# MDAnalysis/transport-analysis

Measured on AMD Instinct MI355X. Metric: VACF lag-points/sec (n_frames x n_atoms / s), higher is better.
Workload: dtype f64

## Files before the change

transport_analysis_amd/csrc/wfft.hpp:

```cpp
#pragma once
#include <hip/hip_runtime.h>

#include <type_traits>
#include <utility>

#include "fft_engine.hpp"

namespace ta {

#ifndef WF_NW_R0
#define WF_NW_R0 0
#define WF_NW_VAL 0
#endif

template <int LO, int HI, class F>
__device__ __forceinline__ void static_for_range(F&& f) {
    [&]<int... I>(std::integer_sequence<int, I...>) {
        (f(std::integral_constant<int, LO + I>{}), ...);
    }(std::make_integer_sequence<int, (HI > LO ? HI - LO : 0)>{});
}

typedef unsigned int wf_u32x4 __attribute__((ext_vector_type(4)));

#include "wfft_twist.inc"
// ... 341 lines not shown
        for (int n2 = 0; n2 < 8; ++n2) v[n2] = reg[64 * n2 + lane];
    }
    __device__ __forceinline__ void stage_a(cd* __restrict__ reg, cd (&v)[8], const cd (&twa)[7]) const {
        Dft<8>::run(v);
#pragma unroll
        for (int a = 1; a < 8; ++a) v[a] = cmul(v[a], twa[a - 1]);
        __builtin_amdgcn_wave_barrier();
#pragma unroll
        for (int a = 0; a < 8; ++a) reg[a * 64 + (lane ^ (8 * (a & 1)))] = v[a];
        __builtin_amdgcn_wave_barrier();
        const int base = hi * 64 + (lo ^ (8 * (hi & 1)));
#pragma unroll
        for (int n1 = 0; n1 < 8; ++n1) v[n1] = reg[base ^ (8 * n1)];
        __builtin_amdgcn_wave_barrier();
    }
    __device__ __forceinline__ void stage_b(cd* __restrict__ reg, cd (&v)[8], const cd (&twb)[7]) const {
        Dft<8>::run(v);
#pragma unroll
        for (int b = 1; b < 8; ++b) v[b] = cmul(v[b], twb[b - 1]);
        __builtin_amdgcn_wave_barrier();
        const int x = lo ^ hi;
#pragma unroll
        for (int b = 0; b < 8; ++b) reg[(hi * 8 + b) * 8 + (x ^ b)] = v[b];
        __builtin_amdgcn_wave_barrier();
#pragma unroll
        for (int n0 = 0; n0 < 8; ++n0) v[n0] = reg[lane * 8 + (n0 ^ x)];
        __builtin_amdgcn_wave_barrier();
    }
    __device__ __forceinline__ void stage_c(cd (&v)[8], double (&acc)[8]) const {
        Dft<8>::run(v);
#pragma unroll
        for (int c = 0; c < 8; ++c) acc[c] = fma(v[c].y, v[c].y, fma(v[c].x, v[c].x, acc[c]));
        __builtin_amdgcn_wave_barrier();
    }
};

template <int ROT>
__device__ __forceinline__ void wf_bf(cd& A, cd& B, const cd t) {
    const double qx = fma(-t.x, B.y, B.x), qy = fma(t.x, B.x, B.y);
    const cd a = A;
    if constexpr (ROT == 0) {
        A = cd{fma(t.y, qx, a.x), fma(t.y, qy, a.y)};
        B = cd{fma(-t.y, qx, a.x), fma(-t.y, qy, a.y)};
    } else {
        A = cd{fma(t.y, qy, a.x), fma(-t.y, qx, a.y)};
        B = cd{fma(-t.y, qy, a.x), fma(t.y, qx, a.y)};
    }
}
__device__ __forceinline__ void wf_dft8_tw(cd (&v)[8], const cd (&t)[4]) {
    wf_bf<0>(v[0], v[4], t[0]);
    wf_bf<0>(v[1], v[5], t[0]);
    wf_bf<0>(v[2], v[6], t[0]);
    wf_bf<0>(v[3], v[7], t[0]);
    wf_bf<0>(v[0], v[2], t[1]);
    wf_bf<0>(v[1], v[3], t[1]);
    wf_bf<1>(v[4], v[6], t[1]);
    wf_bf<1>(v[5], v[7], t[1]);
    wf_bf<0>(v[0], v[1], t[2]);
    wf_bf<1>(v[2], v[3], t[2]);
    wf_bf<0>(v[4], v[5], t[3]);
    wf_bf<1>(v[6], v[7], t[3]);
    const cd y4 = v[1], y6 = v[3], y1 = v[4], y3 = v[6];
    v[1] = y1, v[3] = y3, v[4] = y4, v[6] = y6;
}

struct WfTw {
    cd b[4], c[4];
};
typedef unsigned wf_u32pair __attribute__((ext_vector_type(2)));
__device__ __forceinline__ void wf_transpose_hi(cd (&v)[8]) {
    unsigned w[8][4];
#pragma unroll
    for (int a = 0; a < 8; ++a) {
        const wf_u32x4 t = __builtin_bit_cast(wf_u32x4, v[a]);
        w[a][0] = t.x, w[a][1] = t.y, w[a][2] = t.z, w[a][3] = t.w;
    }
#pragma unroll
    for (int a = 0; a < 8; ++a)
        if (!(a & 4))
#pragma unroll
            for (int d = 0; d < 4; ++d) {
                const wf_u32pair r = __builtin_amdgcn_permlane32_swap(w[a][d], w[a | 4][d], false, false);
                w[a][d] = r.x, w[a | 4][d] = r.y;
            }
#pragma unroll
    for (int a = 0; a < 8; ++a)
        if (!(a & 2))
#pragma unroll
            for (int d = 0; d < 4; ++d) {
                const wf_u32pair r = __builtin_amdgcn_permlane16_swap(w[a][d], w[a | 2][d], false, false);
                w[a][d] = r.x, w[a | 2][d] = r.y;
            }
#pragma unroll
    for (int a = 0; a < 8; ++a)
        if (!(a & 1))
#pragma unroll
            for (int d = 0; d < 4; ++d) {
                const unsigned lo = w[a][d], hi = w[a | 1][d];
                w[a][d] = __builtin_amdgcn_update_dpp(lo, hi, 0x128, 0xF, 0xC, false);
                w[a | 1][d] = __builtin_amdgcn_update_dpp(hi, lo, 0x128, 0xF, 0x3, false);
            }
#pragma unroll
    for (int a = 0; a < 8; ++a) {
        wf_u32x4 t;
        t.x = w[a][0], t.y = w[a][1], t.z = w[a][2], t.w = w[a][3];
        v[a] = __builtin_bit_cast(cd, t);
    }
}

struct WfAddr {
    unsigned we, wo, re, ro, x16, b2w, b2r;
    __device__ __forceinline__ void init(int lane, unsigned q_bytes) {
        const int hi = lane >> 3, lo = lane & 7;
        we = q_bytes + 16u * (unsigned)lane;
        wo = q_bytes + 16u * (unsigned)(lane ^ 8);
        const unsigned rb = q_bytes + 16u * (unsigned)(hi * 64 + lo);
        re = rb + 128u * (unsigned)(hi & 1);
        ro = rb - 128u * (unsigned)(hi & 1);
        x16 = 16u * (unsigned)(hi ^ lo);
        b2w = q_bytes + 1024u * (unsigned)hi;
        b2r = b2w + 128u * (unsigned)lo;
    }
    __device__ __forceinline__ unsigned w2(int k) const { return (x16 ^ (16u * (unsigned)k)) + b2w; }
    __device__ __forceinline__ unsigned r2(int k) const { return (x16 ^ (16u * (unsigned)k)) + b2r; }
};
struct WfSub {
    const WfAddr& ad;
    unsigned char* smem;
    __device__ __forceinline__ WfSub(const WfAddr& ad_, unsigned char* smem_) : ad(ad_), smem(smem_) {}
    __device__ __forceinline__ cd& at(unsigned base, unsigned off) const {
        return *reinterpret_cast<cd*>(__builtin_assume_aligned(smem + (base + off), 16));
    }
    template <unsigned SO>
    __device__ __forceinline__ void read_a(cd (&v)[8]) const {
#pragma unroll
        for (int n2 = 0; n2 < 8; ++n2) v[n2] = at(ad.we, SO + 1024u * n2);
    }
    template <unsigned SO>
    __device__ __forceinline__ void stage_a_w(cd (&v)[8]) const {
        Dft<8>::run(v);
        __builtin_amdgcn_wave_barrier();
#pragma unroll
        for (int a = 0; a < 8; ++a) at(a & 1 ? ad.wo : ad.we, SO + 1024u * a) = v[a];
        __builtin_amdgcn_wave_barrier();
    }
    template <unsigned SO>
    __device__ __forceinline__ void stage_a_r(cd (&v)[8]) const {
        __builtin_amdgcn_wave_barrier();
#pragma unroll
        for (int n1 = 0; n1 < 8; ++n1) v[n1] = at(n1 & 1 ? ad.ro : ad.re, SO + 128u * n1);
        __builtin_amdgcn_wave_barrier();
    }
    template <unsigned SO, bool XV = false>
    __device__ __forceinline__ void stage_a(cd (&v)[8]) const {
        if constexpr (XV) {
            Dft<8>::run(v);
            wf_transpose_hi(v);
        } else {
            stage_a_w<SO>(v);
            stage_a_r<SO>(v);
        }
    }
    template <unsigned SO>
    __device__ __forceinline__ void stage_b_w(cd (&v)[8], const WfTw& tw) const {
        wf_dft8_tw(v, tw.b);
        __builtin_amdgcn_wave_barrier();
#pragma unroll
        for (int b = 0; b < 8; ++b) at(ad.w2(b), SO + 128u * b) = v[b];
        __builtin_amdgcn_wave_barrier();
    }
    template <unsigned SO>
    __device__ __forceinline__ void stage_b_r(cd (&v)[8]) const {
        __builtin_amdgcn_wave_barrier();
#pragma unroll
        for (int n0 = 0; n0 < 8; ++n0) v[n0] = at(ad.r2(n0), SO);
        __builtin_amdgcn_wave_barrier();
    }
    template <unsigned SO>
    __device__ __forceinline__ void stage_b(cd (&v)[8], const WfTw& tw) const {
        stage_b_w<SO>(v, tw);
        stage_b_r<SO>(v);
    }
    __device__ __forceinline__ void stage_c(cd (&v)[8], const WfTw& tw, double (&acc)[8]) const {
        wf_dft8_tw(v, tw.c);
#pragma unroll
        for (int c = 0; c < 8; ++c) acc[c] = fma(v[c].y, v[c].y, fma(v[c].x, v[c].x, acc[c]));
    }
    __device__ __forceinline__ void stage_c_w(cd (&v)[8], const WfTw& tw, double (&acc)[8], double wgt) const {
        wf_dft8_tw(v, tw.c);
#pragma unroll
        for (int c = 0; c < 8; ++c) acc[c] = fma(wgt, fma(v[c].y, v[c].y, v[c].x * v[c].x), acc[c]);
    }
};

constexpr unsigned kWfSubBytes = 512 * sizeof(cd);

struct WfNoHook {
    template <class T>
    __device__ __forceinline__ void operator()(T) const {}
};
template <int I>
using wf_part = std::integral_constant<int, I>;

template <int S0, bool XV = false, class Hook = WfNoHook>
__device__ __forceinline__ void wf_sub512(const WfSub& w, const WfTw& tw, double (&acc)[8], Hook&& hook = Hook{}) {
    cd v[8];
    w.read_a<S0 * kWfSubBytes>(v);
    hook(wf_part<0>{});
    w.template stage_a<S0 * kWfSubBytes, XV>(v);
    hook(wf_part<1>{});
    w.stage_b<S0 * kWfSubBytes>(v, tw);
    hook(wf_part<2>{});
    w.stage_c(v, tw, acc);
    hook(wf_part<3>{});
}

template <int S0, bool XV = false>
__device__ __forceinline__ void wf_sub512_w(const WfSub& w, const WfTw& tw, double (&acc)[8], double wgt) {
    cd v[8];
    w.read_a<S0 * kWfSubBytes>(v);
    w.template stage_a<S0 * kWfSubBytes, XV>(v);
    w.stage_b<S0 * kWfSubBytes>(v, tw);
    w.stage_c_w(v, tw, acc, wgt);
}

template <int S0, bool XV = false, class Hook = WfNoHook>
__device__ __forceinline__ void wf_sub512_x2(const WfSub& w, const WfTw& tw, double (&acc0)[8],
                                             double (&acc1)[8], Hook&& hook = Hook{}) {
    constexpr unsigned A = S0 * kWfSubBytes, B = A + kWfSubBytes;
    cd v0[8], v1[8];
    w.read_a<A>(v0);
    w.read_a<B>(v1);
    __builtin_amdgcn_wave_barrier();
    hook(wf_part<0>{});
    w.template stage_a<A>(v0);
    w.template stage_a<B, XV>(v1);
    hook(wf_part<1>{});
    w.stage_b<A>(v0, tw);
    w.stage_b<B>(v1, tw);
    hook(wf_part<2>{});
    w.stage_c(v0, tw, acc0);
    w.stage_c(v1, tw, acc1);
    hook(wf_part<3>{});
}

template <bool XV = false, class Hook = WfNoHook>
__device__ __forceinline__ void wf_sub512_x3(const WfSub& w, const WfTw& tw, double (&acc0)[8],
                                             double (&acc1)[8], double (&acc2)[8], Hook&& hook = Hook{}) {
    constexpr unsigned A = 0, B = kWfSubBytes, C = 2 * kWfSubBytes;
    cd v0[8], v1[8], v2[8];
    w.read_a<A>(v0);
    w.read_a<B>(v1);
    w.read_a<C>(v2);
    __builtin_amdgcn_wave_barrier();
    hook(wf_part<0>{});
    w.template stage_a<A>(v0);
    w.template stage_a<B>(v1);
    w.template stage_a<C, XV>(v2);
    hook(wf_part<1>{});
    w.stage_b<A>(v0, tw);
    w.stage_b<B>(v1, tw);
    w.stage_b<C>(v2, tw);
    hook(wf_part<2>{});
    w.stage_c(v0, tw, acc0);
    w.stage_c(v1, tw, acc1);
    w.stage_c(v2, tw, acc2);
    hook(wf_part<3>{});
}

__device__ __forceinline__ void wf_unit_of(long atom, int k, int D, long* pair, int* kind) {
    const long c0 = atom * D;
    if (D == 2) {
        *pair = atom, *kind = 2;
    } else if (D == 1) {
        *pair = c0 >> 1, *kind = (int)(c0 & 1);
    } else if ((c0 & 1) == 0) {
        *pair = (c0 >> 1) + k, *kind = k == 0 ? 2 : 0;
    } else {
        *pair = (c0 >> 1) + k, *kind = k == 0 ? 1 : 2;
    }
}

typedef unsigned int wf_u32x2 __attribute__((__vector_size__(2 * sizeof(unsigned int))));

__device__ __forceinline__ cd wf_cfma(cd acc, cd a, cd b) {
    return {acc.x + (a.x * b.x - a.y * b.y), acc.y + (a.x * b.y + a.y * b.x)};
}

template <bool S, class A, class B>
__device__ __forceinline__ auto& wf_pick(A& a, B& b) {
    if constexpr (S) return a;
    else return b;
}

#ifndef WF_PASS_SPLIT
#define WF_PASS_SPLIT 1
#endif
#ifndef WF_SEED_DERIVE
#define WF_SEED_DERIVE 2
#endif
#ifndef WF_TWIST_FOLD
#define WF_TWIST_FOLD 1
#endif
template <class P, bool BYP, bool LONG, bool SRC32>
constexpr bool wf_pass_split = WF_PASS_SPLIT && !BYP && !LONG && !SRC32 && (P::R0 == 18 || P::R0 == 20);

__device__ __forceinline__ cd wf_csqr(cd a) { return {a.x * a.x - a.y * a.y, 2.0 * (a.x * a.y)}; }

template <class P, bool BYP, bool LONG, bool STAMP, bool SRC32, int PASS>
__device__ __forceinline__ void wf_accum_body(unsigned char* smem_raw, const double* __restrict__ pm, long pitch, int T,
                                              long n_units, const cd* __restrict__ tw2, double* __restrict__ accg, int D,
                                              int R_arg, unsigned long long* __restrict__ stamps) {
    cd* lds = reinterpret_cast<cd*>(smem_raw);
    constexpr int R0 = P::R0, N1 = P::N1, NW = P::NW, NS1 = P::NS1, M = P::M;
    static_assert(!(SRC32 && LONG), "float32 slabs: plans without an outer radix only");
    static_assert(PASS < 0 || (!BYP && !LONG), "a compile-time pass: lag sums without an outer radix");
    const int R = LONG ? R_arg : 1, npass = 2 * R, L = npass * M;
    const int tid = threadIdx.x, wave = tid >> 6;
    int lane = tid & 63;
    const int bi = blockIdx.x >> 3;
    const int pass = PASS >= 0 ? PASS : bi % npass;
    constexpr bool kTwistFold = PASS == 1 && WF_TWIST_FOLD && DftTwisted<R0>::kHave;
    const long tuple = (blockIdx.x & 7) + 8 * (bi / npass), n_tuples = gridDim.x / npass;
    const int upa = BYP ? (D == 3 ? 2 : 1) : 1;
    const int grp = BYP && (D & 1) ? 2 : 1;

    double acc[NS1][8];
#pragma unroll
    for (int s = 0; s < NS1; ++s)
#pragma unroll
        for (int c = 0; c < 8; ++c) acc[s][c] = 0.0;
    unsigned long long st_acc[4] = {0, 0, 0, 0}, st_prev = 0, st_t0 = 0, st_r0 = 0, st_tail = 0, st_s2end = 0;
    if constexpr (STAMP) {
        st_prev = st_t0 = __builtin_amdgcn_s_memtime();
        st_r0 = __builtin_amdgcn_s_memrealtime();
    }
#define WF_STAMP(i)                                                   \
    if constexpr (STAMP) {                                            \
        const unsigned long long now_ = __builtin_amdgcn_s_memtime(); \
        st_acc[i] += now_ - st_prev;                                  \
        st_prev = now_;                                               \
    }
    const __amdgpu_buffer_rsrc_t twr =
        __builtin_amdgcn_make_buffer_rsrc(const_cast<cd*>(tw2), 0, (L + kWfStageRows * 64) * 16, 0x00020000);
    auto unit_rsrc = [&](long item, int k, int* kind) {
        long pair = item;
        const bool live = item < n_units;
        *kind = 2;
        if constexpr (BYP) wf_unit_of(live ? item : 0, k, D, &pair, kind);
        if constexpr (SRC32)
            return __builtin_amdgcn_make_buffer_rsrc(
                const_cast<float*>(reinterpret_cast<const float*>(pm) + (live ? pair : 0) * pitch * 2), 0,
                live ? T * 8 : 0, 0x00020000);
        else
            return __builtin_amdgcn_make_buffer_rsrc(const_cast<double*>(pm + (live ? pair : 0) * pitch * 2), 0,
                                                     live ? T * 16 : 0, 0x00020000);
    };
    using RowT = std::conditional_t<SRC32, wf_u32x2, cd>;
    auto load_row = [&](__amdgpu_buffer_rsrc_t rs, int kd, int u, unsigned row_off) -> RowT {
        if constexpr (SRC32) {
            return __builtin_amdgcn_raw_buffer_load_b64(rs, (unsigned)u * 8u, row_off * 8u, 0);
        } else {
            if (!BYP || kd == 2) return wf_load(rs, (unsigned)u * 16u, row_off * 16u);
            return cd{__builtin_bit_cast(double, __builtin_amdgcn_raw_buffer_load_b64(
                                                     rs, (unsigned)u * 16u + (unsigned)kd * 8u, row_off * 16u, 0)),
                      0.0};
        }
    };
    [[maybe_unused]] auto wf_widen = [&](wf_u32x2 r, int kd) {
        if (!BYP || kd == 2)
            return cd{(double)__builtin_bit_cast(float, (unsigned)r[0]), (double)__builtin_bit_cast(float, (unsigned)r[1])};
        return cd{(double)__builtin_bit_cast(float, (unsigned)(kd ? r[1] : r[0])), 0.0};
    };
    constexpr int K1 = P::K1, NT = P::NT;
    RowT xx[K1][R0];
    auto issue_loads = [&](__amdgpu_buffer_rsrc_t rs, int kd) {
#pragma unroll
        for (int k1 = 0; k1 < K1; ++k1) {
            const int u = tid + NT * k1;
            if (K1 * NT != N1 && u >= N1) continue;
            if (!BYP || kd == 2) {
#pragma unroll
                for (int j = 0; j < R0; ++j) xx[k1][j] = load_row(rs, 2, u, (unsigned)(N1 * j));
            } else {
#pragma unroll
                for (int j = 0; j < R0; ++j) xx[k1][j] = load_row(rs, kd, u, (unsigned)(N1 * j));
            }
        }
    };
#ifndef WF_LOAD_PARTS
#define WF_LOAD_PARTS 4
#endif
    constexpr int NR = K1 * R0;
    constexpr bool kSpread = P::kSpreadRows || (SRC32 && R0 >= 18);
#ifndef WF_SPREAD32_TAIL
#define WF_SPREAD32_TAIL 0
#endif
    constexpr int NSPREAD = WF_LOAD_PARTS != 4 ? 0 : (kSpread ? (SRC32 && R0 >= 18 ? NR - WF_SPREAD32_TAIL : NR) : 0);
    auto issue_row = [&](auto ii, __amdgpu_buffer_rsrc_t rs, int kd) {
        constexpr int i = decltype(ii)::value, k1 = i / R0, j = i % R0;
        const int u = tid + NT * k1;
        if (K1 * NT != N1 && u >= N1) return;
        if (!BYP || kd == 2) xx[k1][j] = load_row(rs, 2, u, (unsigned)(N1 * j));
        else xx[k1][j] = load_row(rs, kd, u, (unsigned)(N1 * j));
    };
    auto issue_loads_part = [&](auto part_c, __amdgpu_buffer_rsrc_t rs, int kd) {
        constexpr int PART = decltype(part_c)::value;
        static_for_range<PART * NSPREAD / 4, (PART + 1) * NSPREAD / 4>([&](auto ii) { issue_row(ii, rs, kd); });
    };
    auto issue_loads_tail = [&](__amdgpu_buffer_rsrc_t rs, int kd) {
        static_for_range<NSPREAD, NR>([&](auto ii) { issue_row(ii, rs, kd); });
    };
    int kind = 2, nkind = 2;
    __amdgpu_buffer_rsrc_t crs = unit_rsrc(tuple * grp, 0, &kind);
    issue_loads(crs, kind);
    WfTw stw;
    auto load_stage_tw = [&]() {
#pragma unroll
        for (int a = 0; a < 4; ++a) {
            stw.b[a] = wf_load(twr, (unsigned)lane * 16u, (unsigned)(L + (14 + a) * 64) * 16u);
            stw.c[a] = wf_load(twr, (unsigned)lane * 16u, (unsigned)(L + (18 + a) * 64) * 16u);
        }
    };
    constexpr bool kTwRes = P::kTwResident && !(BYP && LONG && R0 >= 18);
    if constexpr (kTwRes) load_stage_tw();
    WfAddr wad;
    wad.init(lane, (unsigned)P::sub_base(wave) * kWfSubBytes);
    const WfSub wsub(wad, smem_raw);
    int k = 0;
    bool zero_pending = false;
    for (long item = tuple * grp; item < n_units;) {
#ifndef WF_REAL_S1_SKIP
#define WF_REAL_S1_SKIP 0
#endif
        const unsigned qsel = (WF_REAL_S1_SKIP && BYP && kind != 2) ? P::kRealSel.qmask[pass ? 1 : 0] : ~0u;
#pragma unroll
        for (int k1 = 0; k1 < K1; ++k1) {
        const int u = tid + NT * k1;
        if (K1 * NT != N1 && u >= N1) continue;
        [[maybe_unused]] cd xwide[SRC32 ? R0 : 1];
        if constexpr (SRC32) {
#pragma unroll
            for (int j = 0; j < R0; ++j) xwide[j] = wf_widen(xx[k1][j], kind);
        }
        cd(&x)[R0] = wf_pick<SRC32>(xwide, xx[k1]);
        cd g, g2, h;
        auto load_seeds = [&]() {
            if constexpr (PASS == 1 && WF_SEED_DERIVE >= 1) {
                h = wf_load(twr, (unsigned)u * 16u, 0u);
                g = wf_csqr(h);
            } else {
                g = wf_load(twr, (unsigned)(u * R) * 32u, 0u);
                if (PASS != 0) h = wf_load(twr, (unsigned)(u * pass) * 16u, 0u);
            }
            if constexpr ((PASS == 0 && WF_SEED_DERIVE >= 2) || (PASS == 1 && WF_SEED_DERIVE >= 3)) g2 = wf_csqr(g);
            else g2 = wf_load(twr, (unsigned)(u * R) * 64u, 0u);
        };
        if constexpr (!LONG) load_seeds();
        if constexpr (LONG) {
            const int sj = pass * N1, so = pass * M;
            if (pass) {
                int idx = 0;
#pragma unroll
                for (int j = 1; j < R0; ++j) {
                    idx += sj;
                    idx -= idx >= L ? L : 0;
                    x[j] = cmul(x[j], tw_uniform(tw2, idx));
                }
            }
            auto outer_rows = [&](auto single) {
                int base = 0;
                for (int jo = 1; jo < R; ++jo) {
                    base += so;
                    base -= base >= L ? L : 0;
                    if (jo * M >= T) break;
                    int idx = base;
                    constexpr int NZ = 10;
#pragma unroll
                    for (int j0 = 0; j0 < R0; j0 += NZ) {
                        cd z[NZ];
#pragma unroll
                        for (int i = 0; i < NZ; ++i)
                            if (j0 + i < R0)
                                z[i] = load_row(crs, decltype(single)::value ? kind : 2, u, (unsigned)(N1 * (j0 + i) + M * jo));
#pragma unroll
                        for (int i = 0; i < NZ; ++i)
                            if (j0 + i < R0) {
                                x[j0 + i] = wf_cfma(x[j0 + i], z[i], tw_uniform(tw2, idx));
                                idx += sj;
                                idx -= idx >= L ? L : 0;
                            }
                        __builtin_amdgcn_sched_barrier(0);
                    }
                }
            };
            if (BYP && kind != 2) outer_rows(std::true_type{});
            else outer_rows(std::false_type{});
            __builtin_amdgcn_sched_barrier(0);
            load_seeds();
        } else if (pass) {
            if constexpr (!kTwistFold) {
#pragma unroll
                for (int j = 1; j < R0; ++j) x[j] = cmul(x[j], cd{WfTwist<R0>::re(j), WfTwist<R0>::im(j)});
            }
        }
        if constexpr (kTwistFold) DftTwisted<R0>::run(x);
        else Dft<R0>::run(x);
        {
            cd te, to;
            if constexpr (PASS == 0) {
                te = cd{1.0, 0.0};
                to = g;
            } else {
                te = pass ? h : cd{1.0, 0.0};
                to = pass ? cmul(h, g) : g;
                if (pass) x[0] = cmul(x[0], te);
            }
            if (!(WF_REAL_S1_SKIP && BYP) || (qsel & 1u)) lds[u] = x[0];
            if constexpr (R0 > 1) {
                x[1] = cmul(x[1], to);
                if (!(WF_REAL_S1_SKIP && BYP) || (qsel & 2u)) lds[N1 + u] = x[1];
            }
#pragma unroll
            for (int q = 2; q < R0; ++q) {
                if (q & 1) {
                    to = cmul(to, g2);
                    x[q] = cmul(x[q], to);
                } else {
                    te = (PASS == 0 && q == 2) ? g2 : cmul(te, g2);
                    x[q] = cmul(x[q], te);
                }
                if (!(WF_REAL_S1_SKIP && BYP) || (qsel >> q & 1u)) lds[q * N1 + u] = x[q];
            }
        }
        }
        if constexpr (!kTwRes) {
            asm volatile("" : "+v"(lane));
            load_stage_tw();
        }
        WF_STAMP(0)
        __syncthreads();
        if (BYP && zero_pending) {
#pragma unroll
            for (int s = 0; s < NS1; ++s)
#pragma unroll
                for (int c = 0; c < 8; ++c) acc[s][c] = 0.0;
            zero_pending = false;
        }
        const bool last_of_item = !BYP || k == upa - 1;
        long nitem = item;
        if (last_of_item) {
            if (BYP && grp == 2 && (item & 1) == 0 && item + 1 < n_units) nitem = item + 1;
            else nitem = (item & ~(long)(grp - 1)) + grp * n_tuples;
        }
        const int nk = last_of_item ? 0 : k + 1;
        const __amdgpu_buffer_rsrc_t nrs = unit_rsrc(nitem, nk, &nkind);
        auto row_hook = [&](auto part_c) {
#if WF_LOAD_PARTS == 4
            issue_loads_part(part_c, nrs, nkind);
#endif
        };
        if (BYP && kind != 2) {
            const int wv = __builtin_amdgcn_readfirstlane(wave);
            static_for_range<0, 4>([&](auto part_c) { row_hook(part_c); });
            const unsigned qs = P::kRealSel.qmask[pass ? 1 : 0] >> P::sub_base(wv);
            const unsigned q1 = P::kRealSel.q1mask[pass ? 1 : 0] >> P::sub_base(wv);
            static_for_range<0, NS1>([&](auto ss) {
                constexpr int s = decltype(ss)::value;
                if ((s < P::NLO || wv < P::REM) && (qs >> s & 1u))
                    wf_sub512_w<s, P::kRegExchangeSingle>(wsub, stw, acc[s], (q1 >> s & 1u) ? 1.0 : 2.0);
            });
        } else
        if constexpr (NS1 == 3 && P::NLO == 2 && P::REM != 0) {
            if constexpr (SRC32) {
                if (wave < P::REM) wf_sub512_x3<P::kRegExchange>(wsub, stw, acc[0], acc[1], acc[2], row_hook);
                else wf_sub512_x2<0, P::kRegExchange>(wsub, stw, acc[0], acc[1], row_hook);
            } else {
                if (wave < P::REM) wf_sub512_x3<P::kRegExchange>(wsub, stw, acc[0], acc[1], acc[2]);
                else wf_sub512_x2<0, P::kRegExchange>(wsub, stw, acc[0], acc[1]);
            }
        } else {
            static_for_range<0, NS1>([&](auto ss) {
                constexpr int s = decltype(ss)::value;
                constexpr bool full = s < P::NLO;
                constexpr bool nfull = s + 1 < P::NLO;
                constexpr bool head = full && nfull && (s % 2 == 0);
                constexpr bool tail = full && s > 0 && (s % 2 == 1);
                if constexpr (head) {
                    if constexpr (s == 0) wf_sub512_x2<s, P::kRegExchange>(wsub, stw, acc[s], acc[s + 1], row_hook);
                    else wf_sub512_x2<s, P::kRegExchange>(wsub, stw, acc[s], acc[s + 1]);
                } else if constexpr (!tail) {
                    if constexpr (s == 0) wf_sub512<s, P::kRegExchangeSingle>(wsub, stw, acc[s], row_hook);
                    else if (full || wave < P::REM) wf_sub512<s, P::kRegExchangeSingle>(wsub, stw, acc[s]);
                }
            });
        }
        if constexpr (STAMP) st_s2end = __builtin_amdgcn_s_memtime();
        const int wv = __builtin_amdgcn_readfirstlane(wave);
        auto store_acc = [&](long row) {
            const __amdgpu_buffer_rsrc_t sr = __builtin_amdgcn_make_buffer_rsrc(
                accg + (row * npass + pass) * (long)M, 0, M * 8, 0x00020000);
#pragma unroll
            for (int s = 0; s < NS1; ++s) {
                const int q = P::sub_base(wv) + s;
                if (s < P::NLO || wv < P::REM) {
#pragma unroll
                    for (int c2 = 0; c2 < 4; ++c2) {
                        const cd two{acc[s][2 * c2], acc[s][2 * c2 + 1]};
                        __builtin_amdgcn_raw_buffer_store_b128(__builtin_bit_cast(wf_u32x4, two), sr, (unsigned)lane * 16u,
                                                               (unsigned)((q * 4 + c2) * 64) * 16u, 0);
                    }
                }
            }
        };
        if constexpr (BYP) {
            if (last_of_item) {
                store_acc(item);
                zero_pending = true;
            }
        } else {
            if (nitem >= n_units) store_acc(tuple);
        }
        __builtin_amdgcn_sched_barrier(0);
        issue_loads_tail(nrs, nkind);
        kind = nkind, item = nitem, k = nk, crs = nrs;
        if constexpr (STAMP) st_tail += __builtin_amdgcn_s_memtime() - st_s2end;
        WF_STAMP(1)
        __syncthreads();
    }
    if constexpr (!BYP) {
        if (tuple * grp >= n_units) {
            const int wv = __builtin_amdgcn_readfirstlane(wave);
            const __amdgpu_buffer_rsrc_t sr = __builtin_amdgcn_make_buffer_rsrc(
                accg + (tuple * npass + pass) * (long)M, 0, M * 8, 0x00020000);
#pragma unroll
            for (int s = 0; s < NS1; ++s) {
                const int q = P::sub_base(wv) + s;
                if (s < P::sub_count(wv)) {
#pragma unroll
                    for (int c2 = 0; c2 < 4; ++c2)
                        __builtin_amdgcn_raw_buffer_store_b128(__builtin_bit_cast(wf_u32x4, cd{0.0, 0.0}), sr,
                                                               (unsigned)lane * 16u, (unsigned)((q * 4 + c2) * 64) * 16u, 0);
                }
            }
        }
    }
    if constexpr (STAMP) {
        st_acc[2] = __builtin_amdgcn_s_memtime() - st_t0;
        st_acc[3] = __builtin_amdgcn_s_memrealtime() - st_r0;
        if (lane == 0 && (wave == 0 || wave == NW / 2)) {
            for (int i = 0; i < 4; ++i) stamps[16 * (long)blockIdx.x + (wave ? 4 : 0) + i] = st_acc[i];
            stamps[16 * (long)blockIdx.x + 8 + (wave ? 1 : 0)] = st_tail;
        }
    }
#undef WF_STAMP
}

template <class P, bool BYP = false, bool LONG = false, bool STAMP = false, bool SRC32 = false>
__global__ void __launch_bounds__(P::NT, P::min_waves(BYP, LONG))
    k_wsplit_accum(const double* __restrict__ pm, long pitch, int T, long n_units,
                   const cd* __restrict__ tw2, double* __restrict__ accg, int D, int R_arg,
                   unsigned long long* __restrict__ stamps) {
    extern __shared__ __attribute__((aligned(16))) unsigned char smem_raw[];
    if constexpr (wf_pass_split<P, BYP, LONG, SRC32>) {
#ifdef WF_FIX_PASS
        wf_accum_body<P, BYP, LONG, STAMP, SRC32, WF_FIX_PASS>(smem_raw, pm, pitch, T, n_units, tw2, accg, D, R_arg, stamps);
        return;
#endif
        if ((blockIdx.x >> 3) & 1)
            wf_accum_body<P, BYP, LONG, STAMP, SRC32, 1>(smem_raw, pm, pitch, T, n_units, tw2, accg, D, R_arg, stamps);
        else
            wf_accum_body<P, BYP, LONG, STAMP, SRC32, 0>(smem_raw, pm, pitch, T, n_units, tw2, accg, D, R_arg, stamps);
    } else {
        wf_accum_body<P, BYP, LONG, STAMP, SRC32, -1>(smem_raw, pm, pitch, T, n_units, tw2, accg, D, R_arg, stamps);
    }
}

struct WfSubT {
    int lane, hi, lo;
    __device__ __forceinline__ explicit WfSubT(int lane_) : lane(lane_) {
        asm volatile("" : "+v"(lane));
        hi = lane >> 3;
        lo = lane & 7;
    }
    __device__ __forceinline__ void run(cd* __restrict__ reg, cd (&v)[8], const cd (&twa)[7],
                                        const cd (&twb)[7]) const {
        Dft<8>::run(v);
#pragma unroll
        for (int n0 = 1; n0 < 8; ++n0) v[n0] = cmul(v[n0], twb[n0 - 1]);
        __builtin_amdgcn_wave_barrier();
        const int x = lo ^ hi;
#pragma unroll
        for (int n0 = 0; n0 < 8; ++n0) reg[(hi * 8 + n0) * 8 + (x ^ n0)] = v[n0];
        __builtin_amdgcn_wave_barrier();
#pragma unroll
        for (int b = 0; b < 8; ++b) v[b] = reg[lane * 8 + (b ^ x)];
        __builtin_amdgcn_wave_barrier();
        Dft<8>::run(v);
        __builtin_amdgcn_wave_barrier();
        const int base = hi * 64 + (lo ^ (8 * (hi & 1)));
#pragma unroll
        for (int n1 = 0; n1 < 8; ++n1) reg[base ^ (8 * n1)] = v[n1];
        __builtin_amdgcn_wave_barrier();
#pragma unroll
        for (int a = 0; a < 8; ++a) v[a] = reg[a * 64 + (lane ^ (8 * (a & 1)))];
        __builtin_amdgcn_wave_barrier();
#pragma unroll
        for (int a = 1; a < 8; ++a) v[a] = cmul(v[a], twa[a - 1]);
        Dft<8>::run(v);
        __builtin_amdgcn_wave_barrier();
#pragma unroll
        for (int n2 = 0; n2 < 8; ++n2) reg[64 * n2 + lane] = v[n2];
        __builtin_amdgcn_wave_barrier();
    }
};



template <class P, bool LONG = false, int PF = 0>
__global__ void __launch_bounds__(P::NT)
    k_winverse(const double* __restrict__ spec, int T, long n_items, const cd* __restrict__ tw2,
               double* __restrict__ out, long ld, int R_arg) {
    extern __shared__ __attribute__((aligned(16))) unsigned char smem_raw[];
    cd* lds = reinterpret_cast<cd*>(smem_raw);
    constexpr int R0 = P::R0, N1 = P::N1, NW = P::NW, NT = P::NT, K1 = P::K1, M = P::M, NSA = P::NS1;
    static_assert(!LONG || PF == 0, "the spectrum prefetch is for the single-transform case");
    static_assert(PF <= NSA, "prefetch depth counts sub-series of a wave");
    const int R = LONG ? R_arg : 1, L = 2 * R * M;
    int tid = threadIdx.x, lane = tid & 63;
    const int wave = tid >> 6;
    const __amdgpu_buffer_rsrc_t twr =
        __builtin_amdgcn_make_buffer_rsrc(const_cast<cd*>(tw2), 0, (L + kWfStageRows * 64) * 16, 0x00020000);
    cd v[NSA][8];
    auto load_spec = [&](long item, int cp, int s) {
        const int wv = __builtin_amdgcn_readfirstlane(wave);
        const int q = wv + NW * s;
        const bool live = item < n_items && q < R0;
        const __amdgpu_buffer_rsrc_t sr = __builtin_amdgcn_make_buffer_rsrc(
            const_cast<double*>(spec + (live ? item : 0) * (long)L + (long)(2 * cp) * M), 0, live ? 2 * M * 8 : 0,
            0x00020000);
#pragma unroll
        for (int c2 = 0; c2 < 4; ++c2) {
            const cd a = wf_load(sr, (unsigned)lane * 16u, (unsigned)((q * 4 + c2) * 64) * 16u);
            const cd b = wf_load(sr, (unsigned)lane * 16u, (unsigned)(M / 2 + (q * 4 + c2) * 64) * 16u);
            v[s][2 * c2] = cd{a.x, b.x};
            v[s][2 * c2 + 1] = cd{a.y, b.y};
        }
    };
    constexpr bool kHoistNorm = !LONG && R0 >= 9;
    double rnorm[kHoistNorm ? K1 : 1][kHoistNorm ? R0 : 1];
    if constexpr (kHoistNorm) {
#pragma unroll
        for (int k1 = 0; k1 < K1; ++k1)
#pragma unroll
            for (int j = 0; j < R0; ++j) {
                const int n = tid + NT * k1 + N1 * j;
                rnorm[k1][j] = n < T ? 1.0 / (2.0 * (double)M * (double)(T - n)) : 0.0;
            }
    }
#pragma unroll
    for (int s = 0; s < PF; ++s) load_spec(blockIdx.x, 0, s);
    for (long item = blockIdx.x; item < n_items; item += gridDim.x) {
        for (int cp = 0; cp < R; ++cp) {
            asm volatile("" : "+v"(tid), "+v"(lane));
            {
                cd twa[7], twb[7];
#pragma unroll
                for (int a = 0; a < 7; ++a) {
                    twa[a] = wf_load(twr, (unsigned)lane * 16u, (unsigned)(L + a * 64) * 16u);
                    twb[a] = wf_load(twr, (unsigned)lane * 16u, (unsigned)(L + (7 + a) * 64) * 16u);
                }
#pragma unroll
                for (int s = PF; s < NSA; ++s) load_spec(item, cp, s);
                const WfSubT wt(lane);
#pragma unroll
                for (int s = 0; s < NSA; ++s) {
                    const int q = wave + NW * s;
                    if (NW * s + NW - 1 < R0 || q < R0) wt.run(lds + q * N1, v[s], twa, twb);
                }
            }
            __syncthreads();
            if constexpr (PF > 0) {
                __builtin_amdgcn_sched_barrier(0);
#pragma unroll
                for (int s = 0; s < PF; ++s) load_spec(item + gridDim.x, 0, s);
                __builtin_amdgcn_sched_barrier(0);
            }
            cd xx[K1][R0];
#pragma unroll
            for (int k1 = 0; k1 < K1; ++k1) {
                const int u = tid + NT * k1;
                if (K1 * NT != N1 && u >= N1) continue;
                cd(&x)[R0] = xx[k1];
                const cd g = wf_load(twr, (unsigned)(u * R) * 32u, 0u), g2 = wf_load(twr, (unsigned)(u * R) * 64u, 0u);
#pragma unroll
                for (int q = 0; q < R0; ++q) x[q] = lds[q * N1 + u];
                cd te = cd{1.0, 0.0}, to = g;
                if constexpr (R0 > 1) x[1] = cmul(x[1], to);
#pragma unroll
                for (int q = 2; q < R0; ++q) {
                    if (q & 1) {
                        to = cmul(to, g2);
                        x[q] = cmul(x[q], to);
                    } else {
                        te = cmul(te, g2);
                        x[q] = cmul(x[q], te);
                    }
                }
                Dft<R0>::run(x);
            }
            __builtin_amdgcn_wave_barrier();
#pragma unroll
            for (int k1 = 0; k1 < K1; ++k1) {
                const int u = tid + NT * k1;
                if (K1 * NT != N1 && u >= N1) continue;
#pragma unroll
                for (int j = 0; j < R0; ++j) lds[u + N1 * j] = xx[k1][j];
            }
            __syncthreads();
            double* o = out + item * ld;
#pragma unroll
            for (int k1 = 0; k1 < K1; ++k1) {
                const int u = tid + NT * k1;
                if (K1 * NT != N1 && u >= N1) continue;
                cd(&x)[R0] = xx[k1];
                const int mu = u == 0 ? 0 : N1 - u;
                if constexpr (!LONG) {
                    const cd h = wf_load(twr, (unsigned)u * 16u, 0u);
#pragma unroll
                    for (int j = 0; j < R0; ++j) {
                        const int n = u + N1 * j;
                        const int jm = u == 0 ? (R0 - j) % R0 : R0 - 1 - j;
                        const cd qm = lds[mu + N1 * jm];
                        const cd w = j == 0 ? h : cmul(h, cd{WfTwist<R0>::re(j), WfTwist<R0>::im(j)});
                        const double ar = 0.5 * (x[j].x + qm.x), br = 0.5 * (x[j].y + qm.y),
                                     bi = -0.5 * (x[j].x - qm.x);
                        const double lagv = ar + (w.x * br - w.y * bi);
                        if constexpr (kHoistNorm) {
                            if (n < T) o[n] = lagv * rnorm[k1][j];
                        } else {
                            if (n < T) o[n] = lagv / (2.0 * (double)M * (double)(T - n));
                        }
                    }
                } else {
                    const int c0 = 2 * cp, c1 = c0 + 1;
                    const cd h0 = wf_load(twr, (unsigned)(u * c0) * 16u, 0u),
                             h1 = wf_load(twr, (unsigned)(u * c1) * 16u, 0u);
                    const bool first = cp == 0, last = cp == R - 1;
                    int j0 = 0, j1 = 0;
#pragma unroll
                    for (int j = 0; j < R0; ++j) {
                        const int jm = u == 0 ? (R0 - j) % R0 : R0 - 1 - j;
                        const cd qm = lds[mu + N1 * jm];
                        const cd qa = cd{0.5 * (x[j].x + qm.x), 0.5 * (x[j].y - qm.y)};
                        const cd qb = cd{0.5 * (x[j].y + qm.y), -0.5 * (x[j].x - qm.x)};
                        int i0 = j0, i1 = j1;
                        for (int jo = 0; jo < R; ++jo) {
                            const int n = u + N1 * j + M * jo;
                            const cd w0 = cmul(h0, tw_uniform(tw2, i0)), w1 = cmul(h1, tw_uniform(tw2, i1));
                            double a = (w0.x * qa.x - w0.y * qa.y) + (w1.x * qb.x - w1.y * qb.y);
                            if (n < T) {
                                if (!first) a += o[n];
                                o[n] = last ? a / ((double)L * (double)(T - n)) : a;
                            }
                            i0 += c0 * M, i0 -= i0 >= L ? L : 0;
                            i1 += c1 * M, i1 -= i1 >= L ? L : 0;
                        }
                        j0 += c0 * N1, j0 -= j0 >= L ? L : 0;
                        j1 += c1 * N1, j1 -= j1 >= L ? L : 0;
                    }
                }
            }
            __syncthreads();
        }
    }
}

struct W1 {
    static constexpr int NT = 256, NWV = 4, M = 512;
    static constexpr size_t kLds = (size_t)NWV * 2 * 512 * sizeof(cd);
};

template <bool SINGLE>
__device__ __forceinline__ void w1_two_passes(cd* __restrict__ regA, cd* __restrict__ regB, int lane,
                                              const cd (&twa)[7], const cd (&twb)[7], const cd (&v)[8],
                                              const cd (&tB)[8], double (&accA)[8], double (&accB)[8]) {
    const WfSubPost w(lane);
    if constexpr (SINGLE) {
        cd a[8];
#pragma unroll
        for (int n2 = 0; n2 < 8; ++n2) a[n2] = v[n2];
        w.stage_a(regA, a, twa);
        w.stage_b(regA, a, twb);
        w.stage_c(a, accA);
        return;
    }
    cd a[8], b[8];
#pragma unroll
    for (int n2 = 0; n2 < 8; ++n2) {
        a[n2] = v[n2];
        b[n2] = cmul(v[n2], tB[n2]);
    }
    w.stage_a(regA, a, twa);
    w.stage_a(regB, b, twa);
    w.stage_b(regA, a, twb);
    w.stage_b(regB, b, twb);
    w.stage_c(a, accA);
    w.stage_c(b, accB);
}

template <bool SINGLE, int PACK>
__global__ void __launch_bounds__(W1::NT)
    k_w1_accum(const double* __restrict__ pm, long pitch, int T, long n_pairs,
               const cd* __restrict__ tw2, double* __restrict__ accg) {
    static_assert(PACK == 1 || (SINGLE && (PACK == 2 || PACK == 4 || PACK == 8)), "packing needs the one-pass form");
    extern __shared__ __attribute__((aligned(16))) unsigned char smem_raw[];
    cd* lds = reinterpret_cast<cd*>(smem_raw);
    const int tid = threadIdx.x, lane = tid & 63, wave = tid >> 6;
    const long gw = (long)blockIdx.x * W1::NWV + wave, nw = (long)gridDim.x * W1::NWV;
    cd* regA = lds + wave * 1024;
    cd* regB = regA + 512;
    const __amdgpu_buffer_rsrc_t twr = __builtin_amdgcn_make_buffer_rsrc(
        const_cast<cd*>(tw2), 0, (2 * W1::M + kWfStageRows * 64) * 16, 0x00020000);
    cd twa[7], twb[7], tB[8];
#pragma unroll
    for (int a = 0; a < 7; ++a) {
        twa[a] = wf_load(twr, (unsigned)lane * 16u, (unsigned)(2 * W1::M + a * 64) * 16u);
        twb[a] = wf_load(twr, (unsigned)lane * 16u, (unsigned)(2 * W1::M + (7 + a) * 64) * 16u);
    }
#pragma unroll
    for (int n2 = 0; n2 < 8; ++n2) tB[n2] = wf_load(twr, (unsigned)lane * 16u, (unsigned)(64 * n2) * 16u);
// ... 161 lines not shown
```

Before: 112.1 billion.

## Mirror twiddle factors across conjugate-symmetric outputs in compile-time pass kernels

```diff
diff --git a/transport_analysis_amd/csrc/wfft.hpp b/transport_analysis_amd/csrc/wfft.hpp
--- a/transport_analysis_amd/csrc/wfft.hpp
+++ b/transport_analysis_amd/csrc/wfft.hpp
@@ -667,6 +667,9 @@
 #ifndef WF_TWIST_FOLD
 #define WF_TWIST_FOLD 1
 #endif
+#ifndef WF_TWIDDLE_MIRROR
+#define WF_TWIDDLE_MIRROR 1
+#endif
 template <class P, bool BYP, bool LONG, bool SRC32>
 constexpr bool wf_pass_split = WF_PASS_SPLIT && !BYP && !LONG && !SRC32 && (P::R0 == 18 || P::R0 == 20);
 
@@ -686,6 +689,7 @@
     const int bi = blockIdx.x >> 3;
     const int pass = PASS >= 0 ? PASS : bi % npass;
     constexpr bool kTwistFold = PASS == 1 && WF_TWIST_FOLD && DftTwisted<R0>::kHave;
+    constexpr bool kMirror = PASS >= 0 && WF_TWIDDLE_MIRROR && R0 % 2 == 0;
     const long tuple = (blockIdx.x & 7) + 8 * (bi / npass), n_tuples = gridDim.x / npass;
     const int upa = BYP ? (D == 3 ? 2 : 1) : 1;
     const int grp = BYP && (D & 1) ? 2 : 1;
@@ -871,7 +875,40 @@
         }
         if constexpr (kTwistFold) DftTwisted<R0>::run(x);
         else Dft<R0>::run(x);
-        {
+        if constexpr (kMirror) {
+            constexpr int H = R0 / 2;
+            cd te, to;
+            if constexpr (PASS == 0) {
+                te = g2;
+                to = g;
+                lds[u] = x[0];
+#pragma unroll
+                for (int q = 1; q <= H; ++q) {
+                    if (q >= 3 && (q & 1)) to = cmul(to, g2);
+                    else if (q >= 3) te = cmul(te, g2);
+                    const cd t = (q & 1) ? to : te;
+                    x[q] = cmul(x[q], t);
+                    lds[q * N1 + u] = x[q];
+                    if (q < H) {
+                        x[R0 - q] = cmulc(x[R0 - q], t);
+                        lds[(R0 - q) * N1 + u] = x[R0 - q];
+                    }
+                }
+            } else {
+                te = h;
+                to = cmul(h, g);
+#pragma unroll
+                for (int q = 0; q < H; ++q) {
+                    if (q >= 2 && (q & 1)) to = cmul(to, g2);
+                    else if (q >= 2) te = cmul(te, g2);
+                    const cd t = (q & 1) ? to : te;
+                    x[q] = cmul(x[q], t);
+                    lds[q * N1 + u] = x[q];
+                    x[R0 - 1 - q] = cmulc(x[R0 - 1 - q], t);
+                    lds[(R0 - 1 - q) * N1 + u] = x[R0 - 1 - q];
+                }
+            }
+        } else {
             cd te, to;
             if constexpr (PASS == 0) {
                 te = cd{1.0, 0.0};
@@ -984,7 +1021,8 @@
                 zero_pending = true;
             }
         } else {
-            if (nitem >= n_units) store_acc(tuple);
+            if constexpr (!kMirror)
+                if (nitem >= n_units) store_acc(tuple);
         }
         __builtin_amdgcn_sched_barrier(0);
         issue_loads_tail(nrs, nkind);
@@ -992,6 +1030,35 @@
         if constexpr (STAMP) st_tail += __builtin_amdgcn_s_memtime() - st_s2end;
         WF_STAMP(1)
         __syncthreads();
+    }
+    if constexpr (kMirror) {
+        if (tuple * grp < n_units) {
+            const int wv = __builtin_amdgcn_readfirstlane(wave);
+            const __amdgpu_buffer_rsrc_t sr = __builtin_amdgcn_make_buffer_rsrc(
+                accg + (tuple * npass + pass) * (long)M, 0, M * 8, 0x00020000);
+            int ln = (int)__builtin_amdgcn_mbcnt_hi(~0u, __builtin_amdgcn_mbcnt_lo(~0u, 0u));
+            asm volatile("" : "+v"(ln));
+            const unsigned lm = (unsigned)(ln >= 8 ? ln - 8 : ln ? ln + 55 : 63) * 16u;
+#pragma unroll
+            for (int s = 0; s < NS1; ++s) {
+                const int q = P::sub_base(wv) + s;
+                if (s < P::NLO || wv < P::REM) {
+                    const bool mir = PASS == 0 ? q > R0 / 2 : q >= R0 / 2;
+                    const bool carry = mir && ln == 0;
+                    const unsigned ld = mir ? lm : (unsigned)ln * 16u;
+                    const unsigned v0 = ld + (carry ? 3080u : 0u);
+                    const unsigned ve = ld + (carry ? 8u : 1024u);
+                    const unsigned vo = ld + (carry ? 0u : 8u);
+#pragma unroll
+                    for (int cc = 0; cc < 8; ++cc) {
+                        const unsigned at = (unsigned)((cc >> 1) * 64 * 16 + (cc & 1) * 8);
+                        __builtin_amdgcn_raw_buffer_store_b64(__builtin_bit_cast(wf_u32x2, acc[s][cc]), sr,
+                                                              cc == 0 ? v0 : (cc & 1) ? vo + (at - 8u) : ve + (at - 1024u),
+                                                              (unsigned)(q * 4 * 64) * 16u, 0);
+                    }
+                }
+            }
+        }
     }
     if constexpr (!BYP) {
         if (tuple * grp >= n_units) {
```

New measurement: 114.1 billion, median of 6. 1.8% higher.
